# AHupuJR/REFID

Measured on AMD Instinct MI355X. Metric: interpolated frames/sec (train step) GoPro 256x256 11+1, higher is better.
Workload: dtype f32

## Files before the change

### refid_amd/csrc/wgrad_wino24.hip

```cpp
#include "common.h"
#include "wgrad_args.h"
#include <cstdlib>
#include <cstring>
#include <type_traits>
#include <vector>

#ifndef REFID_W24_ABLATE
#define REFID_W24_ABLATE 0
#endif
#define W24_NO_DMA (REFID_W24_ABLATE == 1 || REFID_W24_ABLATE == 5 || REFID_W24_ABLATE == 6)
#define W24_NO_MFMA (REFID_W24_ABLATE == 2)
#define W24_NO_LDS (REFID_W24_ABLATE == 3 || REFID_W24_ABLATE == 6)
#define W24_NO_BAR (REFID_W24_ABLATE == 4 || REFID_W24_ABLATE == 5 || REFID_W24_ABLATE == 6)

namespace {

__device__ __forceinline__ float w24_fake(float seed) { asm volatile("" : "+v"(seed)); return seed; }

constexpr int IT = 32;
constexpr int TC = 4;
constexpr int GH = 4, GW = 4 * TC;
constexpr int XH = GH + 2, XW = GW + 2;
constexpr int X_BYTES = XH * XW * IT * 4;
constexpr int GS_BYTES = GH * GW * 32 * 4;
constexpr int buf_bytes(int ns) { return X_BYTES + ns * GS_BYTES; }
constexpr int lds24_bytes(int ns) { return 2 * buf_bytes(ns); }
constexpr int NXI = 24;
typedef __attribute__((address_space(3))) void* lds_ptr24;
typedef __attribute__((address_space(3))) const float lds_cf24;
typedef float f32x2 __attribute__((ext_vector_type(2)));

template <int AH, int BH>
__device__ __forceinline__ f32x2 w24_pair(f32x2 a, f32x2 b) {
    f32x2 d;
    if constexpr (AH == 0 && BH == 0) asm("v_pk_mov_b32 %0, %1, %2 op_sel:[0,0]" : "=v"(d) : "v"(a), "v"(b));
    else if constexpr (AH == 1 && BH == 0) asm("v_pk_mov_b32 %0, %1, %2 op_sel:[1,0]" : "=v"(d) : "v"(a), "v"(b));
    else if constexpr (AH == 0 && BH == 1) asm("v_pk_mov_b32 %0, %1, %2 op_sel:[0,1]" : "=v"(d) : "v"(a), "v"(b));
    else asm("v_pk_mov_b32 %0, %1, %2 op_sel:[1,1]" : "=v"(d) : "v"(a), "v"(b));
    return d;
}

struct W24Args {
    const float* g[REFID_WGRAD_MAX_GROUPS]; const float* inA[REFID_WGRAD_MAX_GROUPS]; const float* inB[REFID_WGRAD_MAX_GROUPS];
    int groups;
    int ldG, Co;
    int ldA, ldB, Ca, Ctot;
    float* slabs; float* bslabs;
    int N, H, W, Ho, Wo, pad;
    int tilesX, tilesY, ntiles, nsplit;
    int CoP, CiP;
    int accum;
    int Hin, Win, ncoT;
};

template <int I>
struct W24Row {
    static constexpr int XR = XW * IT, GR = GW * 32, GSUB = GH * GW * 32;
    static constexpr int XA = I == 0 ? 0 : (I == 2 ? 2 : (I == 3 ? 3 : 1));
    static constexpr int XB = I == 0 ? 2 : (I == 2 ? 1 : (I == 3 ? 1 : 2));
    static constexpr bool XPLUS = I == 1;

    template <class T>
    static __device__ __forceinline__ T x_comb(T a, T b) { return XPLUS ? a + b : a - b; }
    static __device__ __forceinline__ void x_rows(lds_cf24* const (&xb)[4], int s, f32x2 (&t)[6]) {
#pragma unroll
        for (int c = 0; c < 4; ++c) {
            const int col = 4 * s + 2 + c;
            lds_cf24* p = xb[col & 3] + (col & ~3) * IT;
            const f32x2 a = W24_NO_LDS ? f32x2{w24_fake(1.f + c), w24_fake(2.f)} : f32x2{p[XA * XR], p[XA * XR + 4 * IT]};
            const f32x2 b = W24_NO_LDS ? f32x2{w24_fake(3.f + c), w24_fake(4.f)} : f32x2{p[XB * XR], p[XB * XR + 4 * IT]};
            t[2 + c] = x_comb(a, b);
        }
    }
    static __device__ __forceinline__ f32x2 x_rows01(lds_cf24* xe) {
        if (W24_NO_LDS) return f32x2{w24_fake(5.f), w24_fake(6.f)};
        return x_comb(f32x2{xe[XA * XR], xe[XA * XR + IT]}, f32x2{xe[XB * XR], xe[XB * XR + IT]});
    }
    static __device__ __forceinline__ void g_rows(lds_cf24* const (&gb)[4], int s, int sub, f32x2 (&x)[4]) {
#pragma unroll
        for (int c = 0; c < 4; ++c) {
            const int col = 4 * s + c;
            lds_cf24* p = gb[col & 3] + sub * GSUB + (col & ~3) * 32;
            if (W24_NO_LDS) { x[c] = f32x2{w24_fake(7.f + c), w24_fake(8.f + sub)}; continue; }
            if constexpr (I == 0) x[c] = f32x2{p[0], p[4 * 32]};
            else if constexpr (I == 3) x[c] = f32x2{p[GR], p[GR + 4 * 32]};
            else {
                const f32x2 g0 = f32x2{p[0], p[4 * 32]}, g1 = f32x2{p[GR], p[GR + 4 * 32]};
                x[c] = I == 1 ? g0 + g1 : g0 - g1;
            }
        }
    }
    static __device__ __forceinline__ void v_cols(const f32x2 (&t)[6], f32x2 (&v)[6]) {
        v[0] = 4.f * t[0] + (-5.f * t[2] + t[4]);
        v[1] = (t[3] + t[4]) - 4.f * (t[1] + t[2]);
        v[2] = 4.f * (t[1] - t[2]) + (t[4] - t[3]);
        const f32x2 d42 = t[4] - t[2], d31 = t[3] - t[1];
        v[3] = 2.f * d31 + d42;
        v[4] = d42 - 2.f * d31;
        v[5] = 4.f * t[1] + (-5.f * t[3] + t[5]);
    }
    static __device__ __forceinline__ void z_cols(const f32x2 (&x)[4], f32x2 (&z)[6]) {
        const f32x2 e = x[0] + x[2], o = x[1] + x[3], e4 = 4.f * x[2] + x[0], o4 = 4.f * x[3] + x[1];
        z[0] = x[0]; z[1] = e + o; z[2] = e - o; z[3] = 2.f * o4 + e4; z[4] = e4 - 2.f * o4; z[5] = x[3];
    }
};

template <int NS, bool DOWN>
__global__ __launch_bounds__(256, NS == 2 ? 2 : 3) void wgrad_wino24_kernel(const W24Args a) {
    constexpr int OT = 32 * NS, BUF_BYTES = buf_bytes(NS), XPS = DOWN ? 2 : 1;
    extern __shared__ __attribute__((aligned(16))) char smem[];
    const int tid = threadIdx.x, lane = tid & 63;
    const int wave = __builtin_amdgcn_readfirstlane(tid >> 6);
    const int li = lane & 31, kh = lane >> 5;
    const int phase = DOWN ? blockIdx.z / a.ncoT : 0, php = phase >> 1, phq = phase & 1;
    const int co0 = (DOWN ? blockIdx.z % a.ncoT : blockIdx.z) * OT, ci0 = blockIdx.y * IT;
    const int split = blockIdx.x;
    const int Hin = DOWN ? a.Hin : a.H, Win = DOWN ? a.Win : a.W;

    const bool xFromA = ci0 < a.Ca || ci0 >= a.Ctot;
    const int xld = xFromA ? a.ldA : a.ldB;
    const long long gpixAll = (long long)a.N * a.Ho * a.Wo, xpixAll = (long long)a.N * Hin * Win;
    const int limG = (int)min(gpixAll * a.ldG * 4, 0x7fffffffLL), limX = (int)min(xpixAll * xld * 4, 0x7fffffffLL);
    const int ntAll = a.ntiles * a.groups;
    const int chunk = (ntAll + a.nsplit - 1) / a.nsplit;
    const int p0 = min(split * chunk, ntAll), p1 = min(p0 + chunk, ntAll);

    int qg, qn, qy, qx;
    {
        int t = p0 < ntAll ? p0 : 0;
        qg = t / a.ntiles; t -= qg * a.ntiles;
        qx = t % a.tilesX; t /= a.tilesX;
        qy = t % a.tilesY; qn = t / a.tilesY;
    }
    const int xq = ci0 + (lane & 7) * 4, xt = ci0 + (lane & 31), gq = co0 + (lane & 7) * 4;
    const int xlc = ((lane >> 3) * XPS * xld + (xFromA ? xq : xq - a.Ca)) * 4;
    const int xlt = ((lane >> 5) * XPS * xld + (xFromA ? xt : xt - a.Ca)) * 4;
    const int glc = ((lane >> 3) * a.ldG + gq) * 4;
    const bool fullch = ci0 + IT <= a.Ctot && co0 + OT <= a.Co;
    constexpr int OOB = 0x7ff00000;
    const int xRowB = XPS * Win * xld * 4, gRowB = a.Wo * a.ldG * 4;
    auto x_origin = [&](int n, int ty, int tx) {
        return ((n * Hin + XPS * (ty * GH - a.pad) + php) * Win + XPS * (tx * GW - a.pad) + phq) * xld * 4;
    };
    const float* gPtr = a.g[qg];
    const float* xPtr = xFromA ? a.inA[qg] : a.inB[qg];
    int xTile = x_origin(qn, qy, qx);
    int gTile = ((qn * a.Ho + qy * GH) * a.Wo + qx * GW) * a.ldG * 4;
    auto request = [&](int buf) {
        const int oy0 = qy * GH, ox0 = qx * GW;
        const int iy0 = oy0 - a.pad, ix0 = ox0 - a.pad;
        const __amdgpu_buffer_rsrc_t rsG = __builtin_amdgcn_make_buffer_rsrc(const_cast<float*>(gPtr), 0, limG, 0x00020000);
        const __amdgpu_buffer_rsrc_t rsX = __builtin_amdgcn_make_buffer_rsrc(const_cast<float*>(xPtr), 0, limX, 0x00020000);
        char* xdst = smem + buf * BUF_BYTES;
        char* gdst = xdst + X_BYTES;
        const bool fast = fullch && ix0 >= 0 && ix0 + XW <= a.W && ox0 + GW <= a.Wo && xld * 8 * XPS * 4 < 0x100000 && a.ldG * 8 * 4 < 0x100000;
        const int q0 = NS == 2 ? (wave < 2 ? wave : 3 * wave - 4) : 2 * (wave - 2), nq = NS == 2 ? (wave < 2 ? 1 : 3) : (wave < 2 ? 0 : 2);
        if (fast) {
#pragma unroll
            for (int k = 0; k < 2; ++k) {
                const int r = wave + 4 * k;
                if (r < XH && !W24_NO_DMA) {
                    const int base = (unsigned)(iy0 + r) < (unsigned)a.H ? xTile + r * xRowB : OOB;
                    char* dst = xdst + r * (XW * IT * 4);
                    __builtin_amdgcn_raw_ptr_buffer_load_lds(rsX, (lds_ptr24)dst, 16, base + xlc, 0, 0, 0);
                    __builtin_amdgcn_raw_ptr_buffer_load_lds(rsX, (lds_ptr24)(dst + 1024), 16, base + 8 * XPS * xld * 4 + xlc, 0, 0, 0);
                    __builtin_amdgcn_raw_ptr_buffer_load_lds(rsX, (lds_ptr24)(dst + 2048), 4, base + 16 * XPS * xld * 4 + xlt, 0, 0, 0);
                }
            }
#pragma unroll
            for (int k = 0; k < 3; ++k) {
                if (k < nq && !W24_NO_DMA) {
                    const int q = q0 + k, r = q & 3, sub = q >> 2;
                    const int base = oy0 + r < a.Ho ? gTile + r * gRowB + sub * 128 : OOB;
                    char* dst = gdst + sub * GS_BYTES + r * (GW * 32 * 4);
                    __builtin_amdgcn_raw_ptr_buffer_load_lds(rsG, (lds_ptr24)dst, 16, base + glc, 0, 0, 0);
                    __builtin_amdgcn_raw_ptr_buffer_load_lds(rsG, (lds_ptr24)(dst + 1024), 16, base + 8 * a.ldG * 4 + glc, 0, 0, 0);
                }
            }
        } else {
            const int l8 = lane >> 3, l32 = lane >> 5;
            const int xbadq = xq < a.Ctot ? 0 : -1, xbadt = xt < a.Ctot ? 0 : -1;
            const int gbad0 = gq < a.Co ? 0 : -1, gbad1 = gq + 32 < a.Co ? 0 : -1;
            const int cx0 = (unsigned)(ix0 + l8) < (unsigned)a.W ? 0 : -1;
            const int cx1 = (unsigned)(ix0 + 8 + l8) < (unsigned)a.W ? 0 : -1;
            const int cxt = (unsigned)(ix0 + 16 + l32) < (unsigned)a.W ? 0 : -1;
            const int cg0 = ox0 + l8 < a.Wo ? 0 : -1, cg1 = ox0 + 8 + l8 < a.Wo ? 0 : -1;
#pragma unroll
            for (int k = 0; k < 2; ++k) {
                const int r = wave + 4 * k;
                if (r < XH && !W24_NO_DMA) {
                    const int rbad = (unsigned)(iy0 + r) < (unsigned)a.H ? 0 : -1;
                    const int base = xTile + r * xRowB;
                    char* dst = xdst + r * (XW * IT * 4);
                    __builtin_amdgcn_raw_ptr_buffer_load_lds(rsX, (lds_ptr24)dst, 16, (base + xlc) | xbadq | rbad | cx0, 0, 0, 0);
                    __builtin_amdgcn_raw_ptr_buffer_load_lds(rsX, (lds_ptr24)(dst + 1024), 16,
                                                             (base + 8 * XPS * xld * 4 + xlc) | xbadq | rbad | cx1, 0, 0, 0);
                    __builtin_amdgcn_raw_ptr_buffer_load_lds(rsX, (lds_ptr24)(dst + 2048), 4,
                                                             (base + 16 * XPS * xld * 4 + xlt) | xbadt | rbad | cxt, 0, 0, 0);
                }
            }
#pragma unroll
            for (int k = 0; k < 3; ++k) {
                if (k < nq && !W24_NO_DMA) {
                    const int q = q0 + k, r = q & 3, sub = q >> 2;
                    const int rbad = oy0 + r < a.Ho ? 0 : -1;
                    const int base = gTile + r * gRowB + sub * 128;
                    const int gbad = sub ? gbad1 : gbad0;
                    char* dst = gdst + sub * GS_BYTES + r * (GW * 32 * 4);
                    __builtin_amdgcn_raw_ptr_buffer_load_lds(rsG, (lds_ptr24)dst, 16, (base + glc) | gbad | rbad | cg0, 0, 0, 0);
                    __builtin_amdgcn_raw_ptr_buffer_load_lds(rsG, (lds_ptr24)(dst + 1024), 16,
                                                             (base + 8 * a.ldG * 4 + glc) | gbad | rbad | cg1, 0, 0, 0);
                }
            }
        }
        if (REFID_W24_ABLATE == 7) return;
        qx += 1;
        if (qx != a.tilesX) {
            xTile += GW * XPS * xld * 4;
            gTile += GW * a.ldG * 4;
        } else {
            qx = 0;
            qy += 1;
            if (qy == a.tilesY) {
                qy = 0;
                qn += 1;
                if (qn == a.N) {
                    qn = 0;
                    qg = min(qg + 1, a.groups - 1);
                    gPtr = a.g[qg];
                    xPtr = xFromA ? a.inA[qg] : a.inB[qg];
                }
            }
            xTile = x_origin(qn, qy, 0);
            gTile = (qn * a.Ho + qy * GH) * a.Wo * a.ldG * 4;
        }
    };

    f32x16 acc[6][NS];
#pragma unroll
    for (int j = 0; j < 6; ++j)
#pragma unroll
        for (int sm = 0; sm < NS; ++sm)
#pragma unroll
            for (int r = 0; r < 16; ++r) acc[j][sm][r] = 0.f;
    float bs[NS];
#pragma unroll
    for (int sm = 0; sm < NS; ++sm) bs[sm] = 0.f;

    static_assert(BUF_BYTES % 256 == 0 && (BUF_BYTES + X_BYTES + (NS - 1) * GS_BYTES + 4 * GW * 32 * 4) / 256 < 256, "ds_read2st64 offset range");
    lds_cf24* xe = (lds_cf24*)smem + (2 * kh) * (XW * IT) + li;
    lds_cf24* ge = (lds_cf24*)(smem + X_BYTES) + (2 * kh) * (GW * 32) + li;
    lds_cf24* xb[4] = {xe, xe + IT, xe + 2 * IT, xe + 3 * IT};
    lds_cf24* gb[4] = {ge, ge + 32, ge + 2 * 32, ge + 3 * 32};
    asm volatile("" : "+v"(xb[0]), "+v"(xb[1]), "+v"(xb[2]), "+v"(xb[3]), "+v"(xe));
    asm volatile("" : "+v"(gb[0]), "+v"(gb[1]), "+v"(gb[2]), "+v"(gb[3]));

    auto kloop = [&](auto TI) {
        constexpr int I = decltype(TI)::value;
        using R = W24Row<I>;
        auto tile = [&](auto BUF) {
            constexpr int BO = decltype(BUF)::value * (BUF_BYTES / 4);
            lds_cf24* xbb[4] = {xb[0] + BO, xb[1] + BO, xb[2] + BO, xb[3] + BO};
            lds_cf24* gbb[4] = {gb[0] + BO, gb[1] + BO, gb[2] + BO, gb[3] + BO};
            f32x2 t[6], p4, p5;
#pragma unroll
            for (int s = 0; s < TC; s += 2) {
                R::x_rows(xbb, s, t);
                if (s == 0) {
                    const f32x2 a01 = R::x_rows01(xe + BO);
                    t[0] = w24_pair<0, 0>(a01, t[4]);
                    t[1] = w24_pair<1, 0>(a01, t[5]);
                } else {
                    t[0] = w24_pair<1, 0>(p4, t[4]);
                    t[1] = w24_pair<1, 0>(p5, t[5]);
                }
                p4 = t[4]; p5 = t[5];
                f32x2 v[6];
                R::v_cols(t, v);
#pragma unroll
                for (int sm = 0; sm < NS; ++sm) {
                    f32x2 x[4], z[6];
                    R::g_rows(gbb, s, sm, x);
                    R::z_cols(x, z);
                    if constexpr (I == 1) bs[sm] += z[1][0] + z[1][1];
#pragma unroll
                    for (int h = 0; h < 2; ++h)
#pragma unroll
                        for (int j = 0; j < 6; ++j) {
                            if (W24_NO_MFMA) { asm volatile("" :: "v"(v[j][h]), "v"(z[j][h])); continue; }
                            acc[j][sm] = __builtin_amdgcn_mfma_f32_32x32x2f32(v[j][h], z[j][h], acc[j][sm], 0, 0, 0);
                        }
                }
            }
        };
        auto sync = [&] {
            __builtin_amdgcn_s_waitcnt(0x0F70);
            if (!W24_NO_BAR) __builtin_amdgcn_s_barrier();
            __builtin_amdgcn_sched_barrier(0);
        };
        const int npairs = (p1 - p0) >> 1;
        if (p0 < p1) request(0);
        for (int i = 0; i < npairs; ++i) {
            sync();
            request(1);
            tile(std::integral_constant<int, 0>{});
            sync();
            if (p0 + 2 * i + 2 < p1) request(0);
            tile(std::integral_constant<int, 1>{});
        }
        if ((p1 - p0) & 1) {
            sync();
            tile(std::integral_constant<int, 0>{});
        }
    };
    switch (wave) {
        case 0: kloop(std::integral_constant<int, 0>{}); break;
        case 1: kloop(std::integral_constant<int, 1>{}); break;
        case 2: kloop(std::integral_constant<int, 2>{}); break;
        default: kloop(std::integral_constant<int, 3>{}); break;
    }

#pragma unroll
    for (int j = 0; j < 6; ++j) {
        float* sl = a.slabs + ((long long)((split * (DOWN ? 4 : 1) + phase) * NXI + wave * 6 + j) * a.CoP) * a.CiP;
#pragma unroll
        for (int sm = 0; sm < NS; ++sm) {
            const int co = co0 + sm * 32 + li;
#pragma unroll
            for (int qd = 0; qd < 4; ++qd) {
                const int ci = ci0 + 8 * qd + 4 * kh;
                f32x4 vv;
#pragma unroll
                for (int k = 0; k < 4; ++k) vv[k] = acc[j][sm][4 * qd + k];
                f32x4* dst = reinterpret_cast<f32x4*>(sl + (long long)co * a.CiP + ci);
                if (a.accum) vv += *dst;
                *dst = vv;
            }
        }
    }
    if (a.bslabs != nullptr && blockIdx.y == 0 && phase == 0 && wave == 1) {
#pragma unroll
        for (int sm = 0; sm < NS; ++sm) {
            const float tot = bs[sm] + __shfl_xor(bs[sm], 32, 64);
            if (kh == 0) {
                float* dst = a.bslabs + (long long)split * a.CoP + co0 + sm * 32 + li;
                *dst = a.accum ? *dst + tot : tot;
            }
        }
    }
}

struct W24rArgs {
    const float* slabs; const float* bslabs; float* dw; float* db;
    int nsplit, Co, Ci, CoP, CiP, iBase, iTotal, perGroup;
    int nsplitW;
    int down;
};

__device__ __forceinline__ void w24_fold_body(const float* __restrict__ slabs, float* __restrict__ part, long long slabFloats,
                                              int nsplit, int S, int piece, int s) {
    const long long off = ((long long)piece * 256 + threadIdx.x) * 4;
    if (off >= slabFloats) return;
    const f32x4* p = reinterpret_cast<const f32x4*>(slabs + off);
    const long long st4 = slabFloats / 4;
    f32x4 a0 = {0.f, 0.f, 0.f, 0.f}, a1 = a0;
    int k = s;
    for (; k + S < nsplit; k += 2 * S) { a0 += p[k * st4]; a1 += p[(k + S) * st4]; }
    if (k < nsplit) a0 += p[k * st4];
    *reinterpret_cast<f32x4*>(part + (long long)s * slabFloats + off) = a0 + a1;
}
__global__ __launch_bounds__(256) void wgrad_wino24_fold_kernel(const float* __restrict__ slabs, float* __restrict__ part,
                                                                long long slabFloats, int nsplit, int S) {
    w24_fold_body(slabs, part, slabFloats, nsplit, S, blockIdx.x, blockIdx.y);
}

constexpr int FOLD_BATCH = 96;
struct FoldJob { const float* slabs; float* part; long long slabFloats; int nsplit, S; };
struct FoldBatch { FoldJob job[FOLD_BATCH]; int blk0[FOLD_BATCH + 1]; int n; };
static_assert(sizeof(FoldBatch) <= 4096, "kernel-argument block");
__global__ __launch_bounds__(256) void wgrad_fold_batch_kernel(const FoldBatch b) {
    int j = 0;
    for (int k = 1; k < b.n; ++k) j = (int)blockIdx.x >= b.blk0[k] ? k : j;
    const FoldJob& f = b.job[j];
    const int blk = (int)blockIdx.x - b.blk0[j];
    const int pieces = (int)((f.slabFloats / 4 + 255) / 256);
    w24_fold_body(f.slabs, f.part, f.slabFloats, f.nsplit, f.S, blk % pieces, blk / pieces);
}
thread_local std::vector<FoldJob> fold_queue;

__device__ __forceinline__ void w24_reduce_body(const W24rArgs& a, const int blk, float* part) {
    const long long plane = (long long)a.CoP * a.CiP;
    const long long slabStride = NXI * plane;
    const int lpe = a.perGroup, eb = 256 / lpe;
    const int el = threadIdx.x % eb, sub = threadIdx.x / eb;
    const long long e = (long long)blk * eb + el;
    const bool live = e < (long long)a.Co * a.Ci;
    const int ci = live ? (int)(e % a.Ci) : 0, co = live ? (int)(e / a.Ci) : 0;
    {
        const float* p = a.slabs + (long long)co * a.CiP + ci;
        float u[NXI];
#pragma unroll
        for (int x = 0; x < NXI; ++x) u[x] = 0.f;
        if (live) {
            for (int k = sub; k < a.nsplitW; k += lpe) {
#pragma unroll
                for (int x = 0; x < NXI; ++x) u[x] += p[k * slabStride + x * plane];
            }
        }
        if (lpe > 1) {
#pragma unroll
            for (int x = 0; x < NXI; ++x) part[threadIdx.x * (NXI + 1) + x] = u[x];
            __syncthreads();
            if (sub == 0) {
                for (int s2 = 1; s2 < lpe; ++s2) {
#pragma unroll
                    for (int x = 0; x < NXI; ++x) u[x] += part[(s2 * eb + el) * (NXI + 1) + x];
                }
            }
        }
        if (live && sub == 0) {
            constexpr float c4 = 0.25f, c6 = 1.f / 6.f, c12 = 1.f / 12.f, c24 = 1.f / 24.f;
            float dg[9];
#pragma unroll
            for (int pp = 0; pp < 3; ++pp) {
                float t[6];
#pragma unroll
                for (int j = 0; j < 6; ++j) {
                    const float m = 0.5f * (u[6 + j] + u[12 + j]), d = 0.5f * (u[6 + j] - u[12 + j]);
                    t[j] = pp == 0 ? u[j] + m : (pp == 1 ? d : m + u[18 + j]);
                }
                const float s12 = t[1] + t[2], d21 = t[2] - t[1], s34 = t[3] + t[4], d34 = t[3] - t[4];
                dg[pp * 3 + 0] = c4 * t[0] - c6 * s12 + c24 * s34;
                dg[pp * 3 + 1] = c6 * d21 + c12 * d34;
                dg[pp * 3 + 2] = c6 * (s34 - s12) + t[5];
            }
            float* dst = a.dw + ((long long)co * a.iTotal + a.iBase + ci) * 9;
#pragma unroll
            for (int k = 0; k < 9; ++k) dst[k] += dg[k];
        }
    }
    if (a.db != nullptr && blk == 0) {
        for (int c2 = threadIdx.x; c2 < a.Co; c2 += 256) {
            float s = 0.f;
            for (int k = 0; k < a.nsplit; ++k) s += a.bslabs[(long long)k * a.CoP + c2];
            a.db[c2] += s;
        }
    }
}

__global__ __launch_bounds__(256) void wgrad_wino24_reduce_kernel(const W24rArgs a) {
    __shared__ float part[256 * (NXI + 1)];
    w24_reduce_body(a, blockIdx.x, part);
}

__device__ __forceinline__ void w24_reduce_down_body(const W24rArgs& a, const int blk) {
    const long long plane = (long long)a.CoP * a.CiP;
    const long long slabStride = 4 * NXI * plane;
    const long long gid = (long long)blk * 256 + threadIdx.x;
    const long long e = gid >> 2;
    const int ph = (int)(gid & 3);
    const bool live = e < (long long)a.Co * a.Ci;
    const int ci = live ? (int)(e % a.Ci) : 0, co = live ? (int)(e / a.Ci) : 0;
    if (live) {
        const float* p = a.slabs + (long long)co * a.CiP + ci + ph * NXI * plane;
        float u[NXI];
#pragma unroll
        for (int x = 0; x < NXI; ++x) u[x] = 0.f;
        for (int k = 0; k < a.nsplitW; ++k) {
#pragma unroll
            for (int x = 0; x < NXI; ++x) u[x] += p[k * slabStride + x * plane];
        }
        constexpr float c4 = 0.25f, c6 = 1.f / 6.f, c12 = 1.f / 12.f, c24 = 1.f / 24.f;
        float* dst = a.dw + ((long long)co * a.iTotal + a.iBase + ci) * 16;
#pragma unroll
        for (int pp = 0; pp < 3; ++pp) {
            const int ky = 2 * pp + (ph >> 1) - 1;
            float t[6];
#pragma unroll
            for (int j = 0; j < 6; ++j) {
                const float m = 0.5f * (u[6 + j] + u[12 + j]), d = 0.5f * (u[6 + j] - u[12 + j]);
                t[j] = pp == 0 ? u[j] + m : (pp == 1 ? d : m + u[18 + j]);
            }
            const float s12 = t[1] + t[2], d21 = t[2] - t[1], s34 = t[3] + t[4], d34 = t[3] - t[4];
            const float r3[3] = {c4 * t[0] - c6 * s12 + c24 * s34, c6 * d21 + c12 * d34, c6 * (s34 - s12) + t[5]};
            if (ky < 0 || ky > 3) continue;
#pragma unroll
            for (int q = 0; q < 3; ++q) {
                const int kx = 2 * q + (ph & 1) - 1;
                if (kx >= 0 && kx <= 3) dst[ky * 4 + kx] += r3[q];
            }
        }
    }
    if (a.db != nullptr && blk == 0) {
        for (int c2 = threadIdx.x; c2 < a.Co; c2 += 256) {
            float sacc = 0.f;
            for (int k = 0; k < a.nsplit; ++k) sacc += a.bslabs[(long long)k * a.CoP + c2];
            a.db[c2] += sacc;
        }
    }
}

__global__ __launch_bounds__(256) void wgrad_wino24_reduce_down_kernel(const W24rArgs a) { w24_reduce_down_body(a, blockIdx.x); }

struct W24rBatch { W24rArgs job[REFID_FINISH_BATCH]; int blk0[REFID_FINISH_BATCH + 1]; int n; };
static_assert(sizeof(W24rBatch) <= 4096, "kernel-argument block");
__global__ __launch_bounds__(256) void wgrad_wino24_reduce_batch_kernel(const W24rBatch b) {
    __shared__ float part[256 * (NXI + 1)];
    int j = 0;
    for (int k = 1; k < b.n; ++k) j = (int)blockIdx.x >= b.blk0[k] ? k : j;
    const int blk = (int)blockIdx.x - b.blk0[j];
    if (b.job[j].down) w24_reduce_down_body(b.job[j], blk);
    else w24_reduce_body(b.job[j], blk, part);
}

struct W24rQueued { W24rArgs r; int nblocks; };
thread_local std::vector<W24rQueued> w24_queue;

struct Geo24 { int ncoT, nciT, tilesX, tilesY, ntiles, nsplit, CoP, CiP; };

int ns_of(const refid_wgrad_desc* d) { return d->c_o <= 32 ? 1 : 2; }
bool is_down(const refid_wgrad_desc* d) { return d->kh == 4; }

Geo24 geo24_of(const refid_wgrad_desc* d) {
    Geo24 g;
    const int OT = 32 * ns_of(d);
    g.ncoT = cdiv(d->c_o, OT);
    const int ci_geo = (d->phase != 0) ? d->i_total - d->i_base : d->c_a + d->c_b;
    g.nciT = cdiv(ci_geo > d->c_a + d->c_b ? ci_geo : d->c_a + d->c_b, IT);
    g.tilesX = cdiv(d->wo, GW);
    g.tilesY = cdiv(d->ho, GH);
    g.ntiles = g.tilesX * g.tilesY * d->n;
    static const int wgs = []() { const char* e = getenv("REFID_W24_WGS"); return e ? atoi(e) : 512; }();
    int want = cdiv(ns_of(d) == 1 ? wgs * 3 / 2 : wgs, g.ncoT * g.nciT * (is_down(d) ? 4 : 1));
    if (want >= 8) want = want / 8 * 8;
    if (want < 1) want = 1;
    if (want > g.ntiles) want = g.ntiles;
    g.nsplit = want;
    g.CoP = g.ncoT * OT;
    g.CiP = g.nciT * IT;
    return g;
}

}

int refid_slab_fold_count(long long slabFloats, int nsplit) {
    if (nsplit < 2) return 0;
    const long long pieces = (slabFloats / 4 + 255) / 256;
    int S = (int)((2048 + pieces - 1) / pieces);
    if (S > 16) S = 16;
    if (S >= nsplit) S = nsplit / 2;
    return S < 1 ? 1 : S;
}
int refid_launch_slab_fold(const float* slabs, float* part, long long slabFloats, int nsplit, int S, hipStream_t st) {
    static const bool batch_folds = !(getenv("REFID_FOLD_BATCH") && getenv("REFID_FOLD_BATCH")[0] == '0');
    if (batch_folds && refid_finish_defer_now()) {
        fold_queue.push_back({slabs, part, slabFloats, nsplit, S});
        return 0;
    }
    hipLaunchKernelGGL(wgrad_wino24_fold_kernel, dim3((unsigned)((slabFloats / 4 + 255) / 256), S), dim3(256), 0, st, slabs, part,
                       slabFloats, nsplit, S);
    REFID_LAUNCH_CHECK("wgrad_slab_fold");
    return 0;
}

int refid_slab_fold_flush(hipStream_t st) {
    size_t at = 0;
    while (at < fold_queue.size()) {
        FoldBatch b;
        memset(&b, 0, sizeof(b));
        int n = 0;
        long long blk = 0;
        for (; n < FOLD_BATCH && at < fold_queue.size(); ++n, ++at) {
            const FoldJob& f = fold_queue[at];
            const long long nb = ((f.slabFloats / 4 + 255) / 256) * f.S;
            if (n > 0 && blk + nb > 0x3fffffffLL) break;
            b.job[n] = f;
            b.blk0[n] = (int)blk;
            blk += nb;
        }
        b.blk0[n] = (int)blk; b.n = n;
        hipLaunchKernelGGL(wgrad_fold_batch_kernel, dim3((unsigned)blk), dim3(256), 0, st, b);
        if (hipGetLastError() != hipSuccess) { fold_queue.clear(); refid_set_error("wgrad_fold_batch: launch failed"); return 1; }
    }
    fold_queue.clear();
    return 0;
}

int refid_wino24_finish_flush(hipStream_t st) {
    size_t at = 0;
    while (at < w24_queue.size()) {
        W24rBatch b;
        memset(&b, 0, sizeof(b));
        int n = 0, blk = 0;
        for (; n < REFID_FINISH_BATCH && at < w24_queue.size(); ++n, ++at) {
            b.job[n] = w24_queue[at].r;
            b.blk0[n] = blk;
            blk += w24_queue[at].nblocks;
        }
        b.blk0[n] = blk; b.n = n;
        hipLaunchKernelGGL(wgrad_wino24_reduce_batch_kernel, dim3(blk), dim3(256), 0, st, b);
        if (hipGetLastError() != hipSuccess) { w24_queue.clear(); refid_set_error("wgrad_wino24_reduce_batch: launch failed"); return 1; }
    }
    w24_queue.clear();
    return 0;
}

namespace {
long long slab_floats(const refid_wgrad_desc* d, const Geo24& g) { return (long long)(is_down(d) ? 4 : 1) * NXI * g.CoP * g.CiP; }
}

size_t refid_wgrad_wino24_workspace_bytes(const refid_wgrad_desc* d) {
    const Geo24 g = geo24_of(d);
    const long long slab = slab_floats(d, g);
    return ((size_t)g.nsplit * slab + (size_t)g.nsplit * g.CoP + (size_t)refid_slab_fold_count(slab, g.nsplit) * slab) * sizeof(float);
}

int refid_wgrad_wino24_launch(const refid_wgrad_desc* d, hipStream_t st) {
    static std::atomic<unsigned long long> attr_done{0}, attr_done1{0}, attr_done2{0}, attr_done3{0};
    if (int rc = refid_lds_attr_once(attr_done, &wgrad_wino24_kernel<2, false>, lds24_bytes(2), "wgrad_wino24")) return rc;
    if (int rc = refid_lds_attr_once(attr_done1, &wgrad_wino24_kernel<1, false>, lds24_bytes(1), "wgrad_wino24<1>")) return rc;
    if (int rc = refid_lds_attr_once(attr_done2, &wgrad_wino24_kernel<2, true>, lds24_bytes(2), "wgrad_wino24<down>")) return rc;
    if (int rc = refid_lds_attr_once(attr_done3, &wgrad_wino24_kernel<1, true>, lds24_bytes(1), "wgrad_wino24<1, down>")) return rc;
    const Geo24 g = geo24_of(d);
    const bool down = is_down(d);
    const long long slab = slab_floats(d, g);
    if (down)
        REFID_CHECK(d->kw == 4 && d->stride == 2 && d->pad == 1 && d->h % 2 == 0 && d->w % 2 == 0 && d->ho == d->h / 2 && d->wo == d->w / 2,
                    "wgrad (algo 7): a 4x4 stride-2 pad-1 conv over an even-sized input");
    REFID_CHECK(d->c_b == 0 || d->c_a % IT == 0, "wgrad (Winograd 2x4 tiles): c_a must be a multiple of %d for two sources", IT);
    REFID_CHECK(d->ld_g % 4 == 0 && d->ld_a % 4 == 0 && (d->c_b == 0 || d->ld_b % 4 == 0) && d->c_o % 4 == 0 &&
                    d->c_a % 4 == 0 && d->c_b % 4 == 0,
                "wgrad (Winograd 2x4 tiles): pitches and channel counts must be multiples of 4 floats (16-byte LDS-DMA pieces)");
    {
        const long long lim = 0x7fffffffLL;
        REFID_CHECK((long long)d->n * d->ho * d->wo * d->ld_g * 4 < lim && (long long)d->n * d->h * d->w * d->ld_a * 4 < lim &&
                        (d->c_b == 0 || (long long)d->n * d->h * d->w * d->ld_b * 4 < lim),
                    "wgrad (Winograd 2x4 tiles): tensor too large for 32-bit buffer offsets (use algo 0)");
    }
    W24Args a;
    const int ngrp = d->groups > 1 ? d->groups : 1;
    REFID_CHECK(ngrp <= REFID_WGRAD_MAX_GROUPS, "wgrad: at most %d grouped time steps", REFID_WGRAD_MAX_GROUPS);
    for (int k = 0; k < REFID_WGRAD_MAX_GROUPS; ++k) {
        const bool on = k > 0 && k < ngrp;
        a.g[k] = k == 0 ? d->g : (on ? d->g_more[k - 1] : d->g);
        a.inA[k] = k == 0 ? d->in_a : (on ? d->in_a_more[k - 1] : d->in_a);
        a.inB[k] = k == 0 ? d->in_b : (on ? d->in_b_more[k - 1] : d->in_b);
        REFID_CHECK(a.g[k] && a.inA[k] && (d->c_b == 0 || a.inB[k]), "wgrad: null tensor pointer in group %d", k);
        REFID_CHECK(((uintptr_t)a.g[k] | (uintptr_t)a.inA[k] | (uintptr_t)(d->c_b ? a.inB[k] : nullptr)) % 16 == 0,
                    "wgrad (Winograd 2x4 tiles): tensors must be 16-byte aligned (group %d)", k);
    }
    a.groups = ngrp;
    a.ldG = d->ld_g; a.Co = d->c_o;
    a.ldA = d->ld_a; a.ldB = d->ld_b;
    a.Ca = d->c_a; a.Ctot = d->c_a + d->c_b;
    a.slabs = d->slabs;
    a.bslabs = d->db ? d->slabs + (size_t)g.nsplit * slab : nullptr;
    a.N = d->n; a.H = d->h; a.W = d->w; a.Ho = d->ho; a.Wo = d->wo; a.pad = d->pad;
    a.Hin = d->h; a.Win = d->w; a.ncoT = g.ncoT;
    if (down) { a.H = d->ho; a.W = d->wo; a.pad = 1; }
    a.tilesX = g.tilesX; a.tilesY = g.tilesY; a.ntiles = g.ntiles; a.nsplit = g.nsplit;
    a.CoP = g.CoP; a.CiP = g.CiP;
    a.accum = (d->phase == 2);
    if (d->phase != 3) {
        if (down) {
            if (ns_of(d) == 1)
                hipLaunchKernelGGL((wgrad_wino24_kernel<1, true>), dim3(g.nsplit, g.nciT, 4 * g.ncoT), dim3(256), lds24_bytes(1), st, a);
            else
                hipLaunchKernelGGL((wgrad_wino24_kernel<2, true>), dim3(g.nsplit, g.nciT, 4 * g.ncoT), dim3(256), lds24_bytes(2), st, a);
        } else if (ns_of(d) == 1)
            hipLaunchKernelGGL((wgrad_wino24_kernel<1, false>), dim3(g.nsplit, g.nciT, g.ncoT), dim3(256), lds24_bytes(1), st, a);
        else
            hipLaunchKernelGGL((wgrad_wino24_kernel<2, false>), dim3(g.nsplit, g.nciT, g.ncoT), dim3(256), lds24_bytes(2), st, a);
        REFID_LAUNCH_CHECK("wgrad_wino24");
    }
    if (d->phase == 1 || d->phase == 2) return 0;
    W24rArgs r;
    r.slabs = a.slabs; r.bslabs = a.bslabs; r.dw = d->dw; r.db = d->db;
    r.nsplit = g.nsplit; r.Co = d->o_real;
    int nred = g.nsplit;
    if (const int S = refid_slab_fold_count(slab, g.nsplit)) {
        const long long slabFloats = slab;
        float* part = d->slabs + (size_t)g.nsplit * slab + (size_t)g.nsplit * g.CoP;
        if (int rc = refid_launch_slab_fold(a.slabs, part, slabFloats, g.nsplit, S, st)) return rc;
        r.slabs = part;
        nred = S;
    }
    r.Ci = (d->phase == 0 && a.Ctot < d->i_total - d->i_base) ? a.Ctot : d->i_total - d->i_base;
    r.CoP = g.CoP; r.CiP = g.CiP; r.iBase = d->i_base; r.iTotal = d->i_total;
    const long long total = (long long)r.Co * r.Ci;
    int lpe = 1;
    while (lpe < 16 && (long long)lpe * 2 * total <= 65536 && lpe * 2 <= nred) lpe *= 2;
    r.perGroup = lpe;
    r.nsplitW = nred;
    r.down = down ? 1 : 0;
    if (refid_finish_defer_now()) {
        for (const W24rQueued& q : w24_queue)
            if (q.r.dw == r.dw && q.r.iBase == r.iBase) {
                if (int rc = refid_slab_fold_flush(st)) return rc;
                if (int rc = refid_wino24_finish_flush(st)) return rc;
                break;
            }
        w24_queue.push_back({r, down ? (int)((total * 4 + 255) / 256) : (int)((total + 256 / lpe - 1) / (256 / lpe))});
        return 0;
    }
    if (down) {
        hipLaunchKernelGGL(wgrad_wino24_reduce_down_kernel, dim3((int)((total * 4 + 255) / 256)), dim3(256), 0, st, r);
        REFID_LAUNCH_CHECK("wgrad_wino24_reduce_down");
        return 0;
    }
    hipLaunchKernelGGL(wgrad_wino24_reduce_kernel, dim3((int)((total + 256 / lpe - 1) / (256 / lpe))), dim3(256), 0, st, r);
    REFID_LAUNCH_CHECK("wgrad_wino24_reduce");
    return 0;
}
```

Before: 515.2.

## Add paired-channel-tile Winograd wgrad kernel sharing gradient tiles across 8 waves

```diff
diff --git a/refid_amd/csrc/wgrad_wino24.hip b/refid_amd/csrc/wgrad_wino24.hip
--- a/refid_amd/csrc/wgrad_wino24.hip
+++ b/refid_amd/csrc/wgrad_wino24.hip
@@ -350,6 +350,270 @@
     }
 }
 
+constexpr int PAIR_STAGES = 3;
+constexpr int PAIR_G0 = 2 * PAIR_STAGES * X_BYTES;
+constexpr int PAIR_LDS_BYTES = PAIR_G0 + PAIR_STAGES * 2 * GS_BYTES;
+
+__device__ __forceinline__ int w24_lane_again() {
+    int l = __builtin_amdgcn_mbcnt_hi(~0u, __builtin_amdgcn_mbcnt_lo(~0u, 0u));
+    asm volatile("" : "+v"(l));
+    return l;
+}
+
+template <bool DOWN>
+__global__ __launch_bounds__(512, 1) void wgrad_wino24_pair_kernel(const W24Args a) {
+    constexpr int NS = 2, OT = 32 * NS, XPS = DOWN ? 2 : 1;
+    extern __shared__ __attribute__((aligned(16))) char smem[];
+    const int tid = threadIdx.x, lane = tid & 63;
+    const int wave = __builtin_amdgcn_readfirstlane(tid >> 6);
+    const int row = wave & 3, hf = wave >> 2;
+    const int li = lane & 31, kh = lane >> 5;
+    const int phase = DOWN ? blockIdx.z / a.ncoT : 0, php = phase >> 1, phq = phase & 1;
+    const int co0 = (DOWN ? blockIdx.z % a.ncoT : blockIdx.z) * OT, ci0 = (2 * blockIdx.y + hf) * IT;
+    const int split = blockIdx.x;
+    const int Hin = DOWN ? a.Hin : a.H, Win = DOWN ? a.Win : a.W;
+
+    const bool xFromA = ci0 < a.Ca || ci0 >= a.Ctot;
+    const int xld = xFromA ? a.ldA : a.ldB;
+    const long long gpixAll = (long long)a.N * a.Ho * a.Wo, xpixAll = (long long)a.N * Hin * Win;
+    const int limG = (int)min(gpixAll * a.ldG * 4, 0x7fffffffLL), limX = (int)min(xpixAll * xld * 4, 0x7fffffffLL);
+    const int ntAll = a.ntiles * a.groups;
+    const int chunk = (ntAll + a.nsplit - 1) / a.nsplit;
+    const int p0 = min(split * chunk, ntAll), p1 = min(p0 + chunk, ntAll);
+
+    int qg, qn, qy, qx;
+    {
+        int t = p0 < ntAll ? p0 : 0;
+        qg = t / a.ntiles; t -= qg * a.ntiles;
+        qx = t % a.tilesX; t /= a.tilesX;
+        qy = t % a.tilesY; qn = t / a.tilesY;
+    }
+    const int xq = ci0 + (lane & 7) * 4, xt = ci0 + (lane & 31), gq = co0 + (lane & 7) * 4;
+    const int xlc = ((lane >> 3) * XPS * xld + (xFromA ? xq : xq - a.Ca)) * 4;
+    const int xlt = ((lane >> 5) * XPS * xld + (xFromA ? xt : xt - a.Ca)) * 4;
+    const int glc = ((lane >> 3) * a.ldG + gq) * 4;
+    const bool fullch = ci0 + IT <= a.Ctot && co0 + OT <= a.Co;
+    constexpr int OOB = 0x7ff00000;
+    const int xRowB = XPS * Win * xld * 4, gRowB = a.Wo * a.ldG * 4;
+    auto x_origin = [&](int n, int ty, int tx) {
+        return ((n * Hin + XPS * (ty * GH - a.pad) + php) * Win + XPS * (tx * GW - a.pad) + phq) * xld * 4;
+    };
+    const float* gPtr = a.g[qg];
+    const float* xPtr = xFromA ? a.inA[qg] : a.inB[qg];
+    int xTile = x_origin(qn, qy, qx);
+    int gTile = ((qn * a.Ho + qy * GH) * a.Wo + qx * GW) * a.ldG * 4;
+    const int xr0 = row < 2 ? 2 * row : row + 2, nxr = row < 2 ? 2 : 1;
+    const int gr0 = 2 * (row - 2);
+    auto request = [&](int st) {
+        const int oy0 = qy * GH, ox0 = qx * GW;
+        const int iy0 = oy0 - a.pad, ix0 = ox0 - a.pad;
+        const __amdgpu_buffer_rsrc_t rsG = __builtin_amdgcn_make_buffer_rsrc(const_cast<float*>(gPtr), 0, limG, 0x00020000);
+        const __amdgpu_buffer_rsrc_t rsX = __builtin_amdgcn_make_buffer_rsrc(const_cast<float*>(xPtr), 0, limX, 0x00020000);
+        char* xdst = smem + (hf * PAIR_STAGES + st) * X_BYTES;
+        char* gdst = smem + PAIR_G0 + st * (2 * GS_BYTES) + hf * GS_BYTES;
+        const bool fast = fullch && ix0 >= 0 && ix0 + XW <= a.W && ox0 + GW <= a.Wo && xld * 8 * XPS * 4 < 0x100000 && a.ldG * 8 * 4 < 0x100000;
+        if (fast) {
+#pragma unroll
+            for (int k = 0; k < 2; ++k) {
+                if (k < nxr && !W24_NO_DMA) {
+                    const int r = xr0 + k;
+                    const int base = (unsigned)(iy0 + r) < (unsigned)a.H ? xTile + r * xRowB : OOB;
+                    char* dst = xdst + r * (XW * IT * 4);
+                    __builtin_amdgcn_raw_ptr_buffer_load_lds(rsX, (lds_ptr24)dst, 16, base + xlc, 0, 0, 0);
+                    __builtin_amdgcn_raw_ptr_buffer_load_lds(rsX, (lds_ptr24)(dst + 1024), 16, base + 8 * XPS * xld * 4 + xlc, 0, 0, 0);
+                    __builtin_amdgcn_raw_ptr_buffer_load_lds(rsX, (lds_ptr24)(dst + 2048), 4, base + 16 * XPS * xld * 4 + xlt, 0, 0, 0);
+                }
+            }
+#pragma unroll
+            for (int k = 0; k < 2; ++k) {
+                if (row >= 2 && !W24_NO_DMA) {
+                    const int r = gr0 + k;
+                    const int base = oy0 + r < a.Ho ? gTile + r * gRowB + hf * 128 : OOB;
+                    char* dst = gdst + r * (GW * 32 * 4);
+                    __builtin_amdgcn_raw_ptr_buffer_load_lds(rsG, (lds_ptr24)dst, 16, base + glc, 0, 0, 0);
+                    __builtin_amdgcn_raw_ptr_buffer_load_lds(rsG, (lds_ptr24)(dst + 1024), 16, base + 8 * a.ldG * 4 + glc, 0, 0, 0);
+                }
+            }
+        } else {
+            const int l8 = lane >> 3, l32 = lane >> 5;
+            const int xbadq = xq < a.Ctot ? 0 : -1, xbadt = xt < a.Ctot ? 0 : -1;
+            const int gbad = gq + hf * 32 < a.Co ? 0 : -1;
+            const int cx0 = (unsigned)(ix0 + l8) < (unsigned)a.W ? 0 : -1;
+            const int cx1 = (unsigned)(ix0 + 8 + l8) < (unsigned)a.W ? 0 : -1;
+            const int cxt = (unsigned)(ix0 + 16 + l32) < (unsigned)a.W ? 0 : -1;
+            const int cg0 = ox0 + l8 < a.Wo ? 0 : -1, cg1 = ox0 + 8 + l8 < a.Wo ? 0 : -1;
+#pragma unroll
+            for (int k = 0; k < 2; ++k) {
+                if (k < nxr && !W24_NO_DMA) {
+                    const int r = xr0 + k;
+                    const int rbad = (unsigned)(iy0 + r) < (unsigned)a.H ? 0 : -1;
+                    const int base = xTile + r * xRowB;
+                    char* dst = xdst + r * (XW * IT * 4);
+                    __builtin_amdgcn_raw_ptr_buffer_load_lds(rsX, (lds_ptr24)dst, 16, (base + xlc) | xbadq | rbad | cx0, 0, 0, 0);
+                    __builtin_amdgcn_raw_ptr_buffer_load_lds(rsX, (lds_ptr24)(dst + 1024), 16,
+                                                             (base + 8 * XPS * xld * 4 + xlc) | xbadq | rbad | cx1, 0, 0, 0);
+                    __builtin_amdgcn_raw_ptr_buffer_load_lds(rsX, (lds_ptr24)(dst + 2048), 4,
+                                                             (base + 16 * XPS * xld * 4 + xlt) | xbadt | rbad | cxt, 0, 0, 0);
+                }
+            }
+#pragma unroll
+            for (int k = 0; k < 2; ++k) {
+                if (row >= 2 && !W24_NO_DMA) {
+                    const int r = gr0 + k;
+                    const int rbad = oy0 + r < a.Ho ? 0 : -1;
+                    const int base = gTile + r * gRowB + hf * 128;
+                    char* dst = gdst + r * (GW * 32 * 4);
+                    __builtin_amdgcn_raw_ptr_buffer_load_lds(rsG, (lds_ptr24)dst, 16, (base + glc) | gbad | rbad | cg0, 0, 0, 0);
+                    __builtin_amdgcn_raw_ptr_buffer_load_lds(rsG, (lds_ptr24)(dst + 1024), 16,
+                                                             (base + 8 * a.ldG * 4 + glc) | gbad | rbad | cg1, 0, 0, 0);
+                }
+            }
+        }
+        if (REFID_W24_ABLATE == 7) return;
+        qx += 1;
+        if (qx != a.tilesX) {
+            xTile += GW * XPS * xld * 4;
+            gTile += GW * a.ldG * 4;
+        } else {
+            qx = 0;
+            qy += 1;
+            if (qy == a.tilesY) {
+                qy = 0;
+                qn += 1;
+                if (qn == a.N) {
+                    qn = 0;
+                    qg = min(qg + 1, a.groups - 1);
+                    gPtr = a.g[qg];
+                    xPtr = xFromA ? a.inA[qg] : a.inB[qg];
+                }
+            }
+            xTile = x_origin(qn, qy, 0);
+            gTile = (qn * a.Ho + qy * GH) * a.Wo * a.ldG * 4;
+        }
+    };
+
+    f32x16 acc[6][NS];
+#pragma unroll
+    for (int j = 0; j < 6; ++j)
+#pragma unroll
+        for (int sm = 0; sm < NS; ++sm)
+#pragma unroll
+            for (int r = 0; r < 16; ++r) acc[j][sm][r] = 0.f;
+
+    static_assert(X_BYTES % 256 == 0 && (PAIR_STAGES * X_BYTES) / 256 < 256 && (PAIR_STAGES * 2 * GS_BYTES) / 256 < 256,
+                  "ds_read2st64 offset range");
+    lds_cf24* xe = (lds_cf24*)(smem + hf * PAIR_STAGES * X_BYTES) + (2 * kh) * (XW * IT) + li;
+    lds_cf24* ge = (lds_cf24*)(smem + PAIR_G0) + (2 * kh) * (GW * 32) + li;
+    lds_cf24* xb[4] = {xe, xe + IT, xe + 2 * IT, xe + 3 * IT};
+    lds_cf24* gb[4] = {ge, ge + 32, ge + 2 * 32, ge + 3 * 32};
+    asm volatile("" : "+v"(xb[0]), "+v"(xb[1]), "+v"(xb[2]), "+v"(xb[3]), "+v"(xe));
+    asm volatile("" : "+v"(gb[0]), "+v"(gb[1]), "+v"(gb[2]), "+v"(gb[3]));
+
+    auto kloop = [&](auto TI) {
+        constexpr int I = decltype(TI)::value;
+        using R = W24Row<I>;
+        float bs[NS];
+#pragma unroll
+        for (int sm = 0; sm < NS; ++sm) bs[sm] = 0.f;
+        auto tile = [&](auto ST) {
+            constexpr int XO = decltype(ST)::value * (X_BYTES / 4), GO = decltype(ST)::value * (2 * GS_BYTES / 4);
+            lds_cf24* xbb[4] = {xb[0] + XO, xb[1] + XO, xb[2] + XO, xb[3] + XO};
+            lds_cf24* gbb[4] = {gb[0] + GO, gb[1] + GO, gb[2] + GO, gb[3] + GO};
+            f32x2 t[6], p4, p5;
+#pragma unroll
+            for (int s = 0; s < TC; s += 2) {
+                R::x_rows(xbb, s, t);
+                if (s == 0) {
+                    const f32x2 a01 = R::x_rows01(xe + XO);
+                    t[0] = w24_pair<0, 0>(a01, t[4]);
+                    t[1] = w24_pair<1, 0>(a01, t[5]);
+                } else {
+                    t[0] = w24_pair<1, 0>(p4, t[4]);
+                    t[1] = w24_pair<1, 0>(p5, t[5]);
+                }
+                p4 = t[4]; p5 = t[5];
+                f32x2 v[6];
+                R::v_cols(t, v);
+#pragma unroll
+                for (int sm = 0; sm < NS; ++sm) {
+                    f32x2 x[4], z[6];
+                    R::g_rows(gbb, s, sm, x);
+                    R::z_cols(x, z);
+                    if constexpr (I == 1) bs[sm] += z[1][0] + z[1][1];
+#pragma unroll
+                    for (int h = 0; h < 2; ++h)
+#pragma unroll
+                        for (int j = 0; j < 6; ++j) {
+                            if (W24_NO_MFMA) { asm volatile("" :: "v"(v[j][h]), "v"(z[j][h])); continue; }
+                            acc[j][sm] = __builtin_amdgcn_mfma_f32_32x32x2f32(v[j][h], z[j][h], acc[j][sm], 0, 0, 0);
+                        }
+                }
+            }
+        };
+        const int n = p1 - p0;
+        auto step = [&](auto ST, int j) {
+            constexpr int S = decltype(ST)::value;
+            if (j + 1 < n) __builtin_amdgcn_s_waitcnt(I < 2 ? 0x0F76 : 0x0F77);
+            else __builtin_amdgcn_s_waitcnt(0x0F70);
+            if (!W24_NO_BAR) __builtin_amdgcn_s_barrier();
+            __builtin_amdgcn_sched_barrier(0);
+            if (j + 2 < n) request((S + 2) % PAIR_STAGES);
+            tile(ST);
+        };
+        if (n > 0) request(0);
+        if (n > 1) request(1);
+        int j = 0;
+        for (; j + 3 <= n; j += 3) {
+            step(std::integral_constant<int, 0>{}, j);
+            step(std::integral_constant<int, 1>{}, j + 1);
+            step(std::integral_constant<int, 2>{}, j + 2);
+        }
+        if (j < n) {
+            step(std::integral_constant<int, 0>{}, j);
+            if (j + 1 < n) step(std::integral_constant<int, 1>{}, j + 1);
+        }
+        if constexpr (I == 1) {
+            if (a.bslabs != nullptr && blockIdx.y == 0 && hf == 0 && phase == 0) {
+                const int le = w24_lane_again();
+#pragma unroll
+                for (int sm = 0; sm < NS; ++sm) {
+                    const float tot = bs[sm] + __shfl_xor(bs[sm], 32, 64);
+                    if ((le >> 5) == 0) {
+                        float* dst = a.bslabs + (long long)split * a.CoP + co0 + sm * 32 + (le & 31);
+                        *dst = a.accum ? *dst + tot : tot;
+                    }
+                }
+            }
+        }
+    };
+    switch (row) {
+        case 0: kloop(std::integral_constant<int, 0>{}); break;
+        case 1: kloop(std::integral_constant<int, 1>{}); break;
+        case 2: kloop(std::integral_constant<int, 2>{}); break;
+        default: kloop(std::integral_constant<int, 3>{}); break;
+    }
+
+    const int le = w24_lane_again(), lie = le & 31, khe = le >> 5;
+#pragma unroll
+    for (int j = 0; j < 6; ++j) {
+        float* sl = a.slabs + ((long long)((split * (DOWN ? 4 : 1) + phase) * NXI + row * 6 + j) * a.CoP) * a.CiP;
+#pragma unroll
+        for (int sm = 0; sm < NS; ++sm) {
+            const int co = co0 + sm * 32 + lie;
+#pragma unroll
+            for (int qd = 0; qd < 4; ++qd) {
+                const int ci = ci0 + 8 * qd + 4 * khe;
+                f32x4 vv;
+#pragma unroll
+                for (int k = 0; k < 4; ++k) vv[k] = acc[j][sm][4 * qd + k];
+                f32x4* dst = reinterpret_cast<f32x4*>(sl + (long long)co * a.CiP + ci);
+                if (a.accum) vv += *dst;
+                *dst = vv;
+            }
+        }
+    }
+}
+
 struct W24rArgs {
     const float* slabs; const float* bslabs; float* dw; float* db;
     int nsplit, Co, Ci, CoP, CiP, iBase, iTotal, perGroup;
@@ -530,7 +794,8 @@
     g.tilesX = cdiv(d->wo, GW);
     g.tilesY = cdiv(d->ho, GH);
     g.ntiles = g.tilesX * g.tilesY * d->n;
-    static const int wgs = []() { const char* e = getenv("REFID_W24_WGS"); return e ? atoi(e) : 512; }();
+    const char* wgsEnv = getenv("REFID_W24_WGS");
+    const int wgs = wgsEnv ? atoi(wgsEnv) : 512;
     int want = cdiv(ns_of(d) == 1 ? wgs * 3 / 2 : wgs, g.ncoT * g.nciT * (is_down(d) ? 4 : 1));
     if (want >= 8) want = want / 8 * 8;
     if (want < 1) want = 1;
@@ -540,6 +805,9 @@
     g.CiP = g.nciT * IT;
     return g;
 }
+
+int pair_mode() { const char* e = getenv("REFID_W24_PAIR"); return e ? atoi(e) : 1; }
+bool pair_fits(const refid_wgrad_desc* d, const Geo24& g) { return ns_of(d) == 2 && g.nciT % 2 == 0; }
 
 }
 
@@ -621,9 +889,16 @@
     if (int rc = refid_lds_attr_once(attr_done1, &wgrad_wino24_kernel<1, false>, lds24_bytes(1), "wgrad_wino24<1>")) return rc;
     if (int rc = refid_lds_attr_once(attr_done2, &wgrad_wino24_kernel<2, true>, lds24_bytes(2), "wgrad_wino24<down>")) return rc;
     if (int rc = refid_lds_attr_once(attr_done3, &wgrad_wino24_kernel<1, true>, lds24_bytes(1), "wgrad_wino24<1, down>")) return rc;
+    static std::atomic<unsigned long long> attr_done4{0}, attr_done5{0};
+    if (int rc = refid_lds_attr_once(attr_done4, &wgrad_wino24_pair_kernel<false>, PAIR_LDS_BYTES, "wgrad_wino24<pair>")) return rc;
+    if (int rc = refid_lds_attr_once(attr_done5, &wgrad_wino24_pair_kernel<true>, PAIR_LDS_BYTES, "wgrad_wino24<pair, down>")) return rc;
     const Geo24 g = geo24_of(d);
     const bool down = is_down(d);
     const long long slab = slab_floats(d, g);
+    const int pmode = pair_mode();
+    const bool pair = pmode != 0 && pair_fits(d, g);
+    REFID_CHECK(pair || pmode != 2, "wgrad (Winograd 2x4 tiles): REFID_W24_PAIR=2, but this launch takes the four-wave form "
+                                    "(c_o <= 32 or an odd number of input-channel tiles)");
     if (down)
         REFID_CHECK(d->kw == 4 && d->stride == 2 && d->pad == 1 && d->h % 2 == 0 && d->w % 2 == 0 && d->ho == d->h / 2 && d->wo == d->w / 2,
                     "wgrad (algo 7): a 4x4 stride-2 pad-1 conv over an even-sized input");
@@ -662,7 +937,12 @@
     a.CoP = g.CoP; a.CiP = g.CiP;
     a.accum = (d->phase == 2);
     if (d->phase != 3) {
-        if (down) {
+        if (pair) {
+            if (down)
+                hipLaunchKernelGGL((wgrad_wino24_pair_kernel<true>), dim3(g.nsplit, g.nciT / 2, 4 * g.ncoT), dim3(512), PAIR_LDS_BYTES, st, a);
+            else
+                hipLaunchKernelGGL((wgrad_wino24_pair_kernel<false>), dim3(g.nsplit, g.nciT / 2, g.ncoT), dim3(512), PAIR_LDS_BYTES, st, a);
+        } else if (down) {
             if (ns_of(d) == 1)
                 hipLaunchKernelGGL((wgrad_wino24_kernel<1, true>), dim3(g.nsplit, g.nciT, 4 * g.ncoT), dim3(256), lds24_bytes(1), st, a);
             else
```

After: 523.3, median of 6. +1.6%, better.
